# DengZhuangSouthRd/simple_tensorflow

Hardware: AMD Instinct MI355X
Metric: images/sec (higher is better)
Workload: dtype bf16; 1 GPU; model=resnet50_v1, global_batch=256, parallelism=dp1

## Files before the change

simple_tensorflow_amd/csrc/kernels/gpu_conv.cc:

```cpp
#include "kernels/gpu_common.h"

namespace stf {
namespace {

struct GpuConvGeom {
  int64_t N, H, W, C, R, S, K, sh, sw, ph, pw, P, Q;
  int64_t M() const { return N * P * Q; }
  int64_t RSC() const { return R * S * C; }
  int64_t RSCp() const { return (RSC() + 63) & ~int64_t(63); }
  bool is_1x1_s1() const {
    return R == 1 && S == 1 && sh == 1 && sw == 1 && ph == 0 && pw == 0;
  }
  StfConvGeom abi() const {
    return StfConvGeom{(int)N,  (int)H,  (int)W,  (int)C,  (int)R, (int)S,
                       (int)sh, (int)sw, (int)ph, (int)pw, (int)P, (int)Q, K};
  }
};

static Status GetConvGeom(const TensorShape& x, const TensorShape& f,
                          const std::vector<int64_t>& strides,
                          const std::string& padding, GpuConvGeom* g) {
  g->N = x.dim_size(0);
  g->H = x.dim_size(1);
  g->W = x.dim_size(2);
// ... 103 lines not shown
                                        s));
      return;
    }
    if (path == kImplicitNT) {
      OP_HIP_OK(ctx, stf_conv2d_fwd_nt(x.raw_data(), w.raw_data(),
                                       y->raw_data(), ZeroPage(), &sg, rscp,
                                       s));
      return;
    }
    Tensor col = x;
    if (!g.is_1x1_s1()) OP_HIP_OK(ctx, Im2Col(ctx, x, g, rscp, &col, s));
    if (!fits_8ph && (g.K & 7) == 0) {
      OP_HIP_OK(ctx, stf_gemm_bf16(col.raw_data(), w.raw_data(), y->raw_data(),
                                   g.M(), g.K, rscp, rscp, g.K, 0, 1, s));
    } else {
      OP_HIP_OK(ctx, TransposeBf16(ctx, w.raw_data(), rscp, g.K, &wt, s));
      OP_HIP_OK(ctx, stf_gemm_bf16_nt(col.raw_data(), wt.raw_data(),
                                      y->raw_data(), g.M(), g.K, rscp, s));
    }
  }

 private:
  std::vector<int64_t> strides_;
  std::string padding_;
};
REGISTER_KERNEL_BUILDER(Name("Conv2D").Device(DEVICE_GPU).TypeConstraint<bfloat16>("T"), GpuConv2DOp);

class GpuConv2DBackpropInputOp : public OpKernel {
 public:
  explicit GpuConv2DBackpropInputOp(OpKernelConstruction* c, bool side = false)
      : OpKernel(c), side_(side) {
    c->GetAttr("strides", &strides_);
    c->GetAttr("padding", &padding_);
  }
  void Compute(OpKernelContext* ctx) override {
    auto in_sizes = IntVector(ctx->input(0));
    const Tensor& w = ctx->input(1);
    const Tensor& dy = ctx->input(2);
    hipStream_t s = GPU_STREAM(ctx);
    TensorShape x_shape(in_sizes);
    GpuConvGeom g;
    OP_REQUIRES_OK(ctx, GetConvGeom(x_shape, w.shape(), strides_, padding_,
                                    &g));
    Tensor* dx = ctx->allocate_output(0, x_shape);
    const void* side = nullptr;
    if (side_) {
      const Tensor& sd = ctx->input(3);
      OP_REQUIRES(ctx, sd.NumElements() == dx->NumElements(),
                  errors::InvalidArgument(
                      "Conv2DBackpropInputAdd: side shape mismatch"));
      side = sd.raw_data();
    }
    if (g.is_1x1_s1() && side && stf_gemm_bf16_8ph_ok(g.M(), g.RSC(), g.K)) {
      OP_HIP_OK(ctx, stf_gemm_bf16_8ph_side(dy.raw_data(), w.raw_data(),
                                            dx->raw_data(), side, g.M(),
                                            g.RSC(), g.K, g.K, g.K, s));
      return;
    }
    if (g.is_1x1_s1()) {
      OP_HIP_OK(ctx, stf_gemm_bf16_nt(dy.raw_data(), w.raw_data(),
                                      dx->raw_data(), g.M(), g.RSC(), g.K, s));
    } else {
      Tensor dcol = ctx->allocate_temp(DT_BFLOAT16,
                                       TensorShape({g.M(), g.RSC()}));
      OP_HIP_OK(ctx, stf_gemm_bf16_nt(dy.raw_data(), w.raw_data(),
                                      dcol.raw_data(), g.M(), g.RSC(), g.K,
                                      s));
      StfConvGeom sg = g.abi();
      OP_HIP_OK(ctx, stf_col2im_bf16(dcol.raw_data(), dx->raw_data(), &sg, s));
    }
    if (side)
      OP_HIP_OK(ctx, stf_binary(B_ADD, DtypeCode(DT_BFLOAT16), dx->raw_data(),
                                side, dx->raw_data(), dx->NumElements(), s));
  }

 private:
  std::vector<int64_t> strides_;
  std::string padding_;
  bool side_;
};
REGISTER_KERNEL_BUILDER(Name("Conv2DBackpropInput").Device(DEVICE_GPU).TypeConstraint<bfloat16>("T").HostMemory("input_sizes"), GpuConv2DBackpropInputOp);

class GpuConv2DBackpropInputAddOp : public GpuConv2DBackpropInputOp {
 public:
  explicit GpuConv2DBackpropInputAddOp(OpKernelConstruction* c)
      : GpuConv2DBackpropInputOp(c, true) {}
};
REGISTER_KERNEL_BUILDER(Name("Conv2DBackpropInputAdd").Device(DEVICE_GPU).TypeConstraint<bfloat16>("T").HostMemory("input_sizes"), GpuConv2DBackpropInputAddOp);

class GpuConv2DBackpropFilterOp : public OpKernel {
 public:
  explicit GpuConv2DBackpropFilterOp(OpKernelConstruction* c) : OpKernel(c) {
    c->GetAttr("strides", &strides_);
    c->GetAttr("padding", &padding_);
  }
  void Compute(OpKernelContext* ctx) override {
    hipStream_t s = GPU_STREAM(ctx);
    const Tensor& x = ctx->input(0);
    auto f_sizes = IntVector(ctx->input(1));
    const Tensor& dy = ctx->input(2);
    TensorShape f_shape(f_sizes);
    GpuConvGeom g;
    OP_REQUIRES_OK(ctx, GetConvGeom(x.shape(), f_shape, strides_, padding_,
                                    &g));
    Tensor* dw = ctx->allocate_output(0, f_shape);
    int64_t rsc = g.RSC();

    bool pad_c = (g.C % 8) != 0 && x.dtype() == DT_BFLOAT16;
    enum { kImplicit, kKMajorGemm, kTransposeGemm } path =
        ImplicitConvEnabled() && !g.is_1x1_s1() &&
                ((g.C % 8) == 0 || pad_c) && (g.K & 7) == 0 &&
                (g.M() & 63) == 0 && ZeroPage()
// ... 147 lines not shown
```

simple_tensorflow_amd/csrc/kernels/gpu_nn.cc:

```cpp
#include "kernels/gpu_common.h"

namespace stf {
namespace {

class GpuBiasAddOp : public OpKernel {
 public:
  using OpKernel::OpKernel;
  void Compute(OpKernelContext* ctx) override {
    const Tensor& x = ctx->input(0);
    const Tensor& b = ctx->input(1);
    Tensor* y = ctx->allocate_output(0, x.shape());
    OP_HIP_OK(ctx, stf_bias_add(DtypeCode(x.dtype()), x.raw_data(),
                                b.raw_data(), y->raw_data(), x.NumElements(),
                                (int)b.NumElements(), GPU_STREAM(ctx)));
  }
};
REGISTER_KERNEL_BUILDER(Name("BiasAdd").Device(DEVICE_GPU).TypeConstraint<float>("T"), GpuBiasAddOp);
REGISTER_KERNEL_BUILDER(Name("BiasAdd").Device(DEVICE_GPU).TypeConstraint<bfloat16>("T"), GpuBiasAddOp);

class GpuBiasAddGradOp : public OpKernel {
 public:
  using OpKernel::OpKernel;
  void Compute(OpKernelContext* ctx) override {
    const Tensor& dy = ctx->input(0);
// ... 150 lines not shown
                                   offset.raw_data(), y->raw_data(), rows, c,
                                   s));
  }

 private:
  float eps_ = 1e-4f;
};
REGISTER_KERNEL_BUILDER(Name("BatchNormAddReluMi").Device(DEVICE_GPU).TypeConstraint<bfloat16>("T"), GpuBatchNormAddReluMiOp);

class GpuBatchNormMiGradOp : public OpKernel {
 public:
  explicit GpuBatchNormMiGradOp(OpKernelConstruction* c) : OpKernel(c) {
    c->GetAttr("fuse_relu", &fuse_relu_);
  }
  void Compute(OpKernelContext* ctx) override {
    const Tensor& dy = ctx->input(0);
    const Tensor& x = ctx->input(1);
    const Tensor& scale = ctx->input(2);
    const Tensor& mean = ctx->input(3);
    const Tensor& inv_std = ctx->input(4);
    const Tensor& y_relu = ctx->input(5);
    int c = (int)x.dim_size(x.dims() - 1);
    int64_t rows = x.NumElements() / c;
    Tensor* dx = ctx->allocate_output(0, x.shape());
    Tensor* dscale = ctx->allocate_output(1, TensorShape({c}));
    Tensor* doffset = ctx->allocate_output(2, TensorShape({c}));
    hipStream_t s = GPU_STREAM(ctx);
    OP_HIP_OK(ctx, ZeroF32(doffset->raw_data(), c, s));
    OP_HIP_OK(ctx, ZeroF32(dscale->raw_data(), c, s));
    OP_HIP_OK(ctx, stf_bn_bwd(DtypeCode(x.dtype()), dy.raw_data(),
                              x.raw_data(), y_relu.raw_data(),
                              mean.flat<float>(), inv_std.flat<float>(),
                              scale.raw_data(), doffset->flat<float>(),
                              dscale->flat<float>(), dx->raw_data(), rows, c,
                              fuse_relu_ ? 1 : 0, s));
  }

 private:
  bool fuse_relu_ = false;
};
class GpuBatchNormAddReluMiGradOp : public OpKernel {
 public:
  using OpKernel::OpKernel;
  void Compute(OpKernelContext* ctx) override {
    const Tensor& dy = ctx->input(0);
    const Tensor& x = ctx->input(1);
    const Tensor& scale = ctx->input(2);
    const Tensor& mean = ctx->input(3);
    const Tensor& inv_std = ctx->input(4);
    const Tensor& y_relu = ctx->input(5);
    int c = (int)x.dim_size(x.dims() - 1);
    int64_t rows = x.NumElements() / c;
    Tensor* dx = ctx->allocate_output(0, x.shape());
    Tensor* dscale = ctx->allocate_output(1, TensorShape({c}));
    Tensor* doffset = ctx->allocate_output(2, TensorShape({c}));
    Tensor* dside = ctx->allocate_output(3, x.shape());
    hipStream_t s = GPU_STREAM(ctx);
    OP_HIP_OK(ctx, ZeroF32(doffset->raw_data(), c, s));
    OP_HIP_OK(ctx, ZeroF32(dscale->raw_data(), c, s));
    OP_HIP_OK(ctx, stf_bn_bwd(DtypeCode(x.dtype()), dy.raw_data(),
                              x.raw_data(), y_relu.raw_data(),
                              mean.flat<float>(), inv_std.flat<float>(),
                              scale.raw_data(), doffset->flat<float>(),
                              dscale->flat<float>(), dx->raw_data(), rows, c,
                              1, s));
    OP_HIP_OK(ctx, stf_binary(B_RELU_GRAD, DtypeCode(x.dtype()),
                              dy.raw_data(), y_relu.raw_data(),
                              dside->raw_data(), x.NumElements(), s));
  }
};
REGISTER_KERNEL_BUILDER(Name("BatchNormAddReluMiGrad").Device(DEVICE_GPU).TypeConstraint<bfloat16>("T"), GpuBatchNormAddReluMiGradOp);

REGISTER_KERNEL_BUILDER(Name("BatchNormMiGrad").Device(DEVICE_GPU).TypeConstraint<float>("T"), GpuBatchNormMiGradOp);
REGISTER_KERNEL_BUILDER(Name("BatchNormMiGrad").Device(DEVICE_GPU).TypeConstraint<bfloat16>("T"), GpuBatchNormMiGradOp);

struct PoolAttrs {
  std::vector<int64_t> ksize, strides;
  std::string padding;
};
static void GetPool(OpKernelConstruction* c, PoolAttrs* p) {
  c->GetAttr("ksize", &p->ksize);
  c->GetAttr("strides", &p->strides);
  c->GetAttr("padding", &p->padding);
}
static StfPoolGeom PoolGeomFor(const TensorShape& x, const PoolAttrs& p) {
  StfPoolGeom g;
  g.N = (int)x.dim_size(0);
  g.H = (int)x.dim_size(1);
  g.W = (int)x.dim_size(2);
  g.C = (int)x.dim_size(3);
  g.kh = (int)p.ksize[1];
  g.kw = (int)p.ksize[2];
  g.sh = (int)p.strides[1];
  g.sw = (int)p.strides[2];
  if (p.padding == "SAME") {
    g.P = (g.H + g.sh - 1) / g.sh;
    g.Q = (g.W + g.sw - 1) / g.sw;
    g.ph = std::max(0, (g.P - 1) * g.sh + g.kh - g.H) / 2;
    g.pw = std::max(0, (g.Q - 1) * g.sw + g.kw - g.W) / 2;
  } else {
    g.P = (g.H - g.kh) / g.sh + 1;
// ... 185 lines not shown
```

simple_tensorflow_amd/csrc/kernels/hip/bn.hip:

```cpp
#include "hip_common.h"
#include "stf_kernels.h"

namespace {

template <typename T>
__global__ void BnStatsKernel(const T* __restrict__ x, float* __restrict__ acc,
                              int64_t rows, int c) {
  extern __shared__ __attribute__((aligned(16))) char smem[];
  float* s1 = (float*)smem;
  float* s2 = s1 + c;
  for (int i = threadIdx.x; i < c; i += blockDim.x) {
    s1[i] = 0.f;
    s2[i] = 0.f;
  }
  __syncthreads();
  int64_t n = rows * c;
  int64_t gstride = (int64_t)gridDim.x * blockDim.x;
  for (int64_t i = (int64_t)blockIdx.x * blockDim.x + threadIdx.x; i < n;
       i += gstride) {
    float f = (float)x[i];
    int ch = (int)(i % c);
    atomicAdd(&s1[ch], f);
    atomicAdd(&s2[ch], f * f);
  }
// ... 40 lines not shown
                                  const T* __restrict__ x,
                                  const T* __restrict__ yr,
                                  const float* __restrict__ mean,
                                  const float* __restrict__ inv_std,
                                  float* __restrict__ sum_dy,
                                  float* __restrict__ sum_dy_xhat,
                                  int64_t rows, int c) {
  extern __shared__ __attribute__((aligned(16))) char smem[];
  float* s1 = (float*)smem;
  float* s2 = s1 + c;
  for (int i = threadIdx.x; i < c; i += blockDim.x) {
    s1[i] = 0.f;
    s2[i] = 0.f;
  }
  __syncthreads();
  int64_t n = rows * c;
  int64_t gstride = (int64_t)gridDim.x * blockDim.x;
  for (int64_t i = (int64_t)blockIdx.x * blockDim.x + threadIdx.x; i < n;
       i += gstride) {
    int ch = (int)(i % c);
    float gf = (float)dy[i];
    if (RELU && (float)yr[i] <= 0.f) gf = 0.f;
    float xhat = ((float)x[i] - mean[ch]) * inv_std[ch];
    atomicAdd(&s1[ch], gf);
    atomicAdd(&s2[ch], gf * xhat);
  }
  __syncthreads();
  for (int i = threadIdx.x; i < c; i += blockDim.x) {
    atomicAdd(&sum_dy[i], s1[i]);
    atomicAdd(&sum_dy_xhat[i], s2[i]);
  }
}

template <typename T, bool RELU>
__global__ void BnGradKernel(const T* __restrict__ dy, const T* __restrict__ x,
                             const T* __restrict__ yr,
                             const float* __restrict__ mean,
                             const float* __restrict__ inv_std,
                             const float* __restrict__ scale,
                             const float* __restrict__ sum_dy,
                             const float* __restrict__ sum_dy_xhat,
                             T* __restrict__ dx, int64_t n, int64_t rows,
                             int c) {
  int64_t stride = (int64_t)gridDim.x * blockDim.x;
  float inv_rows = 1.f / (float)rows;
  for (int64_t i = blockIdx.x * blockDim.x + threadIdx.x; i < n; i += stride) {
    int ch = (int)(i % c);
    float xhat = ((float)x[i] - mean[ch]) * inv_std[ch];
    float g = (float)dy[i];
    if (RELU && (float)yr[i] <= 0.f) g = 0.f;
    dx[i] = (T)(scale[ch] * inv_std[ch] *
                (g - sum_dy[ch] * inv_rows -
                 xhat * sum_dy_xhat[ch] * inv_rows));
  }
}

struct BnIdx {
  int nw;
  int w;
  int64_t chunk;
  int64_t chunks;
  bool active;
};

__device__ __forceinline__ BnIdx BnThreadIndex(int c, int64_t rows) {
  BnIdx ix;
  ix.nw = c >> 3;
  int64_t tid = (int64_t)blockIdx.x * blockDim.x + threadIdx.x;
  int64_t nthreads = (int64_t)gridDim.x * blockDim.x;
  ix.chunks = nthreads / ix.nw;
  if (ix.chunks > rows) ix.chunks = rows;
  if (ix.chunks < 1) ix.chunks = 1;
  ix.w = (int)(tid % ix.nw);
  ix.chunk = tid / ix.nw;
  ix.active = ix.chunk < ix.chunks;
  return ix;
}

inline int BnGridV9(int c, int64_t rows) {
  int nw = c >> 3;
  int64_t chunks = (131072 + nw - 1) / nw;
  if (chunks > rows) chunks = rows;
  if (chunks < 1) chunks = 1;
  return (int)((nw * chunks + 255) / 256) + 1;
}

// ... 132 lines not shown
    for (int e = 0; e < 8; ++e) {
      mloc[e] = mean[cb + e];
      iloc[e] = inv_std[cb + e];
    }
    int64_t off = (int64_t)cb;
    for (int64_t r = ix.chunk; r < rows; r += ix.chunks) {
      __bf16 g[8], xv[8], yv[8];
      Load8(g, dy + r * c + off);
      Load8(xv, x + r * c + off);
      if (RELU) Load8(yv, yr + r * c + off);
#pragma unroll
      for (int e = 0; e < 8; ++e) {
        float gf = (float)g[e];
        if (RELU && (float)yv[e] <= 0.f) gf = 0.f;
        float xhat = ((float)xv[e] - mloc[e]) * iloc[e];
        p1[e] += gf;
        p2[e] += gf * xhat;
      }
    }
#pragma unroll
    for (int e = 0; e < 8; ++e) {
      atomicAdd(&s1[cb + e], p1[e]);
      atomicAdd(&s2[cb + e], p2[e]);
    }
  }
  __syncthreads();
  for (int i = threadIdx.x; i < c; i += blockDim.x)
    if (s1[i] != 0.f || s2[i] != 0.f) {
      atomicAdd(&sum_dy[i], s1[i]);
      atomicAdd(&sum_dy_xhat[i], s2[i]);
    }
}

template <bool RELU>
__global__ void BnGradKernelV9(const __bf16* __restrict__ dy,
                               const __bf16* __restrict__ x,
                               const __bf16* __restrict__ yr,
                               const float* __restrict__ mean,
                               const float* __restrict__ inv_std,
                               const float* __restrict__ scale,
                               const float* __restrict__ sum_dy,
                               const float* __restrict__ sum_dy_xhat,
                               __bf16* __restrict__ dx, int64_t rows, int c) {
  BnIdx ix = BnThreadIndex(c, rows);
  if (!ix.active) return;
  int cb = ix.w * 8;
  float inv_rows = 1.f / (float)rows;
  float m[8], is[8], k[8], a[8], b[8];
#pragma unroll
  for (int e = 0; e < 8; ++e) {
    m[e] = mean[cb + e];
    is[e] = inv_std[cb + e];
    k[e] = scale[cb + e] * is[e];
    a[e] = sum_dy[cb + e] * inv_rows;
    b[e] = sum_dy_xhat[cb + e] * inv_rows;
  }
  for (int64_t r = ix.chunk; r < rows; r += ix.chunks) {
    __bf16 g8[8], x8[8], y8[8], o[8];
    Load8(g8, dy + r * c + cb);
    Load8(x8, x + r * c + cb);
    if (RELU) Load8(y8, yr + r * c + cb);
#pragma unroll
    for (int e = 0; e < 8; ++e) {
      float xhat = ((float)x8[e] - m[e]) * is[e];
      float g = (float)g8[e];
      if (RELU && (float)y8[e] <= 0.f) g = 0.f;
      o[e] = (__bf16)(k[e] * (g - a[e] - xhat * b[e]));
    }
    Store8(dx + r * c + cb, o);
  }
}

inline bool UseV9(int dtype, int c) { return dtype != 0 && c % 8 == 0; }

inline size_t BnLdsBytes(int c) { return (size_t)c * 2 * sizeof(float); }

void LaunchBnStats(int dtype, const void* x, float* acc, float* mean,
                   float* var, float* inv_std, int64_t rows, int c, float eps,
                   hipStream_t stream) {
  if (UseV9(dtype, c)) {
    hipLaunchKernelGGL(BnStatsKernelV9, dim3(BnGridV9(c, rows)), dim3(256),
                       BnLdsBytes(c), stream, (const __bf16*)x, acc, rows, c);
  } else {
    DispatchDtype(dtype, [&](auto t) {
      using T = typename decltype(t)::type;
      hipLaunchKernelGGL((BnStatsKernel<T>), dim3(512), dim3(256),
                         BnLdsBytes(c), stream, (const T*)x, acc, rows, c);
    });
  }
  hipLaunchKernelGGL(BnFinalizeKernel, dim3((c + 255) / 256), dim3(256), 0,
                     stream, acc, mean, var, inv_std, rows, c, eps);
}

}

extern "C" {

hipError_t stf_bn_stats_only(int dtype, const void* x, float* acc, float* mean,
                             float* var, float* inv_std, int64_t rows, int c,
                             float eps, hipStream_t stream) {
  LaunchBnStats(dtype, x, acc, mean, var, inv_std, rows, c, eps, stream);
  return hipGetLastError();
// ... 11 lines not shown
                         dim3(256), 0, stream, (const __bf16*)x, mean,
                         inv_std, (const float*)scale, (const float*)offset,
                         (__bf16*)y, rows, c);
      return;
    }
    DispatchDtype(dtype, [&](auto t) {
      using T = typename decltype(t)::type;
      int64_t n = rows * c;
      hipLaunchKernelGGL((BnNormKernel<T, RELU>), ElemwiseGrid(n, 256, 4),
                         dim3(256), 0, stream, (const T*)x, mean, inv_std,
                         (const float*)scale, (const float*)offset, (T*)y, n,
                         c);
    });
  });
  return hipGetLastError();
}

hipError_t stf_bn_add_relu(const void* x, const void* side, const float* mean,
                           const float* inv_std, const void* scale,
                           const void* offset, void* y, int64_t rows, int c,
                           hipStream_t stream) {
  if (c % 8 != 0) return hipErrorInvalidValue;
  hipLaunchKernelGGL(BnNormAddReluKernelV9, dim3(BnGridV9(c, rows)),
                     dim3(256), 0, stream, (const __bf16*)x,
                     (const __bf16*)side, mean, inv_std, (const float*)scale,
                     (const float*)offset, (__bf16*)y, rows, c);
  return hipGetLastError();
}

hipError_t stf_bn_bwd(int dtype, const void* dy, const void* x,
                      const void* y_relu, const float* mean,
                      const float* inv_std, const void* scale,
                      float* sum_dy, float* sum_dy_xhat, void* dx,
                      int64_t rows, int c, int fuse_relu,
                      hipStream_t stream) {
  DispatchBool(fuse_relu, [&](auto relu) {
    constexpr bool RELU = decltype(relu)::value;
    if (UseV9(dtype, c)) {
      dim3 g9(BnGridV9(c, rows));
      hipLaunchKernelGGL((BnGradStatsKernelV9<RELU>), g9, dim3(256),
                         BnLdsBytes(c), stream, (const __bf16*)dy,
                         (const __bf16*)x, (const __bf16*)y_relu, mean,
                         inv_std, sum_dy, sum_dy_xhat, rows, c);
      hipLaunchKernelGGL((BnGradKernelV9<RELU>), g9, dim3(256), 0, stream,
                         (const __bf16*)dy, (const __bf16*)x,
                         (const __bf16*)y_relu, mean, inv_std,
                         (const float*)scale, sum_dy, sum_dy_xhat,
                         (__bf16*)dx, rows, c);
      return;
    }
    DispatchDtype(dtype, [&](auto t) {
      using T = typename decltype(t)::type;
      int64_t n = rows * c;
      hipLaunchKernelGGL((BnGradStatsKernel<T, RELU>), dim3(512), dim3(256),
                         BnLdsBytes(c), stream, (const T*)dy, (const T*)x,
                         (const T*)y_relu, mean, inv_std, sum_dy, sum_dy_xhat,
                         rows, c);
      hipLaunchKernelGGL((BnGradKernel<T, RELU>), ElemwiseGrid(n, 256, 4),
                         dim3(256), 0, stream, (const T*)dy, (const T*)x,
                         (const T*)y_relu, mean, inv_std,
                         (const float*)scale, sum_dy, sum_dy_xhat, (T*)dx, n,
                         rows, c);
    });
  });
  return hipGetLastError();
}

}
```

simple_tensorflow_amd/csrc/kernels/hip/conv_im2col.hip:

```cpp
#include "hip_common.h"
#include "stf_kernels.h"

namespace {

struct ConvGeom {
  int N, H, W, C, R, S, K, sh, sw, ph, pw, P, Q;
};

__global__ void Im2ColKernel(const __bf16* __restrict__ x,
                             __bf16* __restrict__ col, ConvGeom g,
                             int64_t total_vec, int vec, int64_t ld) {
  int64_t stride = (int64_t)gridDim.x * blockDim.x;
  int64_t cvec = g.C / vec;
  for (int64_t i = blockIdx.x * blockDim.x + threadIdx.x; i < total_vec;
       i += stride) {
    int64_t rem = i;
    int64_t cv = rem % cvec; rem /= cvec;
    int s = (int)(rem % g.S); rem /= g.S;
    int r = (int)(rem % g.R); rem /= g.R;
    int q = (int)(rem % g.Q); rem /= g.Q;
    int p = (int)(rem % g.P); rem /= g.P;
    int n = (int)rem;
    int ih = p * g.sh - g.ph + r;
    int iw = q * g.sw - g.pw + s;
    int64_t m = ((int64_t)(n * g.P + p) * g.Q + q);
    int64_t rsc = ((int64_t)(r * g.S + s) * g.C + cv * vec);
    __bf16* dst = col + m * ld + rsc;
    if (ih >= 0 && ih < g.H && iw >= 0 && iw < g.W) {
      const __bf16* src =
          x + (((int64_t)(n * g.H + ih) * g.W + iw) * g.C + cv * vec);
      if (vec == 8) {
        *(ulong2*)dst = *(const ulong2*)src;
      } else {
        for (int e = 0; e < vec; ++e) dst[e] = src[e];
      }
    } else {
      if (vec == 8) {
        *(ulong2*)dst = ulong2{0, 0};
      } else {
        for (int e = 0; e < vec; ++e) dst[e] = (__bf16)0.f;
      }
    }
  }
}

__global__ void Col2ImKernel(const __bf16* __restrict__ dcol,
                             __bf16* __restrict__ dx, ConvGeom g,
                             int64_t total) {
  int64_t stride = (int64_t)gridDim.x * blockDim.x;
  int64_t RSC = (int64_t)g.R * g.S * g.C;
  for (int64_t i = blockIdx.x * blockDim.x + threadIdx.x; i < total;
       i += stride) {
    int64_t rem = i;
    int c = (int)(rem % g.C); rem /= g.C;
    int iw = (int)(rem % g.W); rem /= g.W;
    int ih = (int)(rem % g.H); rem /= g.H;
    int n = (int)rem;
    float acc = 0.f;
    for (int r = 0; r < g.R; ++r) {
      int ph = ih + g.ph - r;
      if (ph < 0 || ph % g.sh) continue;
      int p = ph / g.sh;
      if (p >= g.P) continue;
      for (int s = 0; s < g.S; ++s) {
        int pw = iw + g.pw - s;
        if (pw < 0 || pw % g.sw) continue;
        int q = pw / g.sw;
        if (q >= g.Q) continue;
        int64_t m = (int64_t)(n * g.P + p) * g.Q + q;
        acc += (float)dcol[m * RSC + (int64_t)(r * g.S + s) * g.C + c];
      }
    }
    dx[i] = (__bf16)acc;
  }
}

__global__ void Col2ImKernelV8(const __bf16* __restrict__ dcol,
                               __bf16* __restrict__ dx, ConvGeom g,
                               int64_t total8) {
  int64_t stride = (int64_t)gridDim.x * blockDim.x;
  int64_t RSC = (int64_t)g.R * g.S * g.C;
  int cg = g.C / 8;
  for (int64_t i = blockIdx.x * blockDim.x + threadIdx.x; i < total8;
       i += stride) {
    int64_t rem = i;
    int c8 = (int)(rem % cg); rem /= cg;
    int iw = (int)(rem % g.W); rem /= g.W;
    int ih = (int)(rem % g.H); rem /= g.H;
    int n = (int)rem;
    float acc[8] = {0, 0, 0, 0, 0, 0, 0, 0};
    for (int r = 0; r < g.R; ++r) {
      int ph = ih + g.ph - r;
      if (ph < 0 || ph % g.sh) continue;
      int p = ph / g.sh;
      if (p >= g.P) continue;
      for (int s = 0; s < g.S; ++s) {
        int pw = iw + g.pw - s;
        if (pw < 0 || pw % g.sw) continue;
        int q = pw / g.sw;
        if (q >= g.Q) continue;
        int64_t m = (int64_t)(n * g.P + p) * g.Q + q;
        __bf16 v[8];
        *(ulong2*)v = *(const ulong2*)(
            dcol + m * RSC + (int64_t)(r * g.S + s) * g.C + c8 * 8);
#pragma unroll
        for (int e = 0; e < 8; ++e) acc[e] += (float)v[e];
      }
    }
    __bf16 out[8];
#pragma unroll
    for (int e = 0; e < 8; ++e) out[e] = (__bf16)acc[e];
    *(ulong2*)(dx + i * 8) = *(ulong2*)out;
  }
}

}

namespace {
ConvGeom DeviceGeom(const StfConvGeom& g) {
  return ConvGeom{g.n, g.h, g.w, g.c, g.r, g.s, 0, g.sh, g.sw, g.ph, g.pw,
                  g.p, g.q};
}
}

extern "C" hipError_t stf_im2col_bf16(const void* x, void* col,
                                      const StfConvGeom* sg, int64_t ld,
                                      hipStream_t stream) {
  ConvGeom g = DeviceGeom(*sg);
  int vec = (g.C % 8 == 0) ? 8 : 1;
  int64_t total = (int64_t)g.N * g.P * g.Q * g.R * g.S * (g.C / vec);
  hipLaunchKernelGGL(Im2ColKernel, ElemwiseGrid(total, 256, 1), dim3(256), 0,
                     stream, (const __bf16*)x, (__bf16*)col, g, total, vec,
                     ld);
  return hipGetLastError();
}

extern "C" hipError_t stf_col2im_bf16(const void* dcol, void* dx,
                                      const StfConvGeom* sg,
                                      hipStream_t stream) {
  ConvGeom g = DeviceGeom(*sg);
  int64_t total = (int64_t)g.N * g.H * g.W * g.C;
  if (g.C % 8 == 0) {
    int64_t total8 = total / 8;
    hipLaunchKernelGGL(Col2ImKernelV8, ElemwiseGrid(total8, 256, 1),
                       dim3(256), 0, stream, (const __bf16*)dcol,
                       (__bf16*)dx, g, total8);
  } else {
    hipLaunchKernelGGL(Col2ImKernel, ElemwiseGrid(total, 256, 1), dim3(256),
                       0, stream, (const __bf16*)dcol, (__bf16*)dx, g, total);
  }
  return hipGetLastError();
}
```

simple_tensorflow_amd/csrc/kernels/hip/gemm_bf16_8ph.hip:

```cpp
#include "hip_common.h"
#include "stf_kernels.h"

#include <type_traits>

namespace {

__device__ __forceinline__ f32x4 mfma_bf16_8(bf16x8 a, bf16x8 b, f32x4 c) {
  return __builtin_amdgcn_mfma_f32_16x16x32_bf16(a, b, c, 0, 0, 0);
}

__device__ __forceinline__ int Swz8(int r) { return (r ^ (r >> 3)) & 7; }

constexpr int kBM = 256, kBK = 64;
constexpr int kThreads = 512;

template <int ROWS, class AG>
__device__ __forceinline__ void Stage8(const AG& ag, int64_t row0, int64_t k0,
                                       uint16_t* lds_base, int tid) {
#pragma unroll
  for (int p = 0; p < ROWS / 64; ++p) {
    int s = p * kThreads + tid;
    int r = s >> 3;
    int c8 = (s & 7) ^ Swz8(r);
    const uint16_t* g = ag.at(row0 + r, k0 + c8 * 8);
// ... 220 lines not shown
  if (N % 256 == 0) launch(std::integral_constant<int, 4>{});
  else if (N % 128 == 0) launch(std::integral_constant<int, 2>{});
  else launch(std::integral_constant<int, 1>{});
  return hipGetLastError();
}

}

extern "C" {

int stf_gemm_bf16_8ph_ok(int64_t M, int64_t N, int64_t K) {
  return (M % 256 == 0) && (N % 64 == 0) && (K % 64 == 0) && K > 0;
}

hipError_t stf_gemm_bf16_8ph_side(const void* A, const void* B, void* C,
                                  const void* side_bf16, int64_t M, int64_t N,
                                  int64_t K, int64_t lda, int64_t ldb,
                                  hipStream_t stream) {
  if (!stf_gemm_bf16_8ph_ok(M, N, K)) return hipErrorInvalidValue;
  LinearAG ag{(const uint16_t*)A, lda};
  return Launch8Ph(ag, B, C, side_bf16, M, N, K, ldb, stream);
}

hipError_t stf_conv2d_fwd_8ph(const void* x, const void* wt, void* y,
                              const void* zero16, const StfConvGeom* g,
                              int64_t rscp, hipStream_t stream) {
  int64_t M = (int64_t)g->n * g->p * g->q;
  if (!stf_gemm_bf16_8ph_ok(M, g->cout, rscp) || (g->c % 8) != 0)
    return hipErrorInvalidValue;
  return Launch8Ph(MakeConvAG(*g, x, zero16), wt, y, nullptr, M, g->cout,
                   rscp, rscp, stream);
}

}
```

simple_tensorflow_amd/csrc/kernels/hip/hip_common.h:

```cpp
#pragma once

#include <hip/hip_runtime.h>

#include <cstdint>
#include <type_traits>

#include "stf_kernels.h"

#define STF_WAVE 64
#define STF_NUM_XCD 8
#define STF_NUM_CU 256

using f32x4 = __attribute__((ext_vector_type(4))) float;
using f32x16 = __attribute__((ext_vector_type(16))) float;
using bf16x8 = __attribute__((ext_vector_type(8))) __bf16;
using bf16x4 = __attribute__((ext_vector_type(4))) __bf16;
using s16x8 = __attribute__((ext_vector_type(8))) short;

__device__ __forceinline__ float bf16_to_f32(uint16_t v) {
  union { uint32_t u; float f; } c;
  c.u = ((uint32_t)v) << 16;
  return c.f;
}

// ... 90 lines not shown
  __device__ __forceinline__ const uint16_t* at(int64_t row,
                                                int64_t k8) const {
    if (k8 >= rsc) return zero16;
    uint32_t row32 = (uint32_t)row, k32 = (uint32_t)k8;
    uint32_t n = div_pq.div(row32);
    uint32_t pq = div_pq.mod(row32, n);
    uint32_t p = div_q.div(pq);
    uint32_t q = div_q.mod(pq, p);
    uint32_t rs = div_c.div(k32);
    uint32_t c = div_c.mod(k32, rs);
    uint32_t r = div_s.div(rs);
    uint32_t s_ = div_s.mod(rs, r);
    int h = (int)p * sh - ph + (int)r;
    int w = (int)q * sw - pw + (int)s_;
    if (h < 0 || h >= H || w < 0 || w >= W) return zero16;
    return x + ((((int64_t)n * H + h) * W + w) * C + c);
  }
};

inline ConvAG MakeConvAG(const StfConvGeom& g, const void* x,
                         const void* zero16) {
  ConvAG ag;
  ag.x = (const uint16_t*)x;
  ag.zero16 = (const uint16_t*)zero16;
  ag.div_pq.init((uint32_t)(g.p * g.q));
  ag.div_q.init((uint32_t)g.q);
  ag.div_c.init((uint32_t)g.c);
  ag.div_s.init((uint32_t)g.s);
  ag.H = g.h; ag.W = g.w; ag.C = g.c; ag.S = g.s;
  ag.sh = g.sh; ag.sw = g.sw; ag.ph = g.ph; ag.pw = g.pw;
  ag.rsc = (int64_t)g.r * g.s * g.c;
  return ag;
}
```

simple_tensorflow_amd/csrc/kernels/hip/stf_kernels.h:

```cpp
#pragma once

#include <hip/hip_runtime_api.h>

#include <cstdint>

struct StfConvGeom {
  int n, h, w, c;
  int r, s;
  int sh, sw, ph, pw;
  int p, q;
  int64_t cout;
};

struct StfPoolGeom {
  int N, H, W, C, kh, kw, sh, sw, ph, pw, P, Q;
};

constexpr int kStfMaxPermuteRank = 6;

enum StfReduce { STF_REDUCE_SUM = 0, STF_REDUCE_MAX = 1, STF_REDUCE_MIN = 2 };
constexpr float StfReduceIdentity(StfReduce kind) {
  return kind == STF_REDUCE_SUM ? 0.f
         : kind == STF_REDUCE_MAX ? -3.4e38f : 3.4e38f;
}

extern "C" {

hipError_t stf_gemm_bf16(const void* A, const void* B, void* C, int64_t M,
                         int64_t N, int64_t K, int64_t lda, int64_t ldb,
                         int a_km, int b_km, hipStream_t stream);
hipError_t stf_gemm_bf16_nt(const void* A, const void* B, void* C, int64_t M,
                            int64_t N, int64_t K, hipStream_t stream);
hipError_t stf_gemm_bf16_splitk(const void* A, const void* B, void* C_f32,
                                int64_t M, int64_t N, int64_t K, int64_t lda,
                                int64_t ldb, int a_km, int b_km, int splitk,
                                hipStream_t stream);
int stf_gemm_bf16_8ph_ok(int64_t M, int64_t N, int64_t K);
hipError_t stf_gemm_bf16_8ph_side(const void* A, const void* B, void* C,
                                  const void* side_bf16, int64_t M, int64_t N,
                                  int64_t K, int64_t lda, int64_t ldb,
                                  hipStream_t stream);
hipError_t stf_gemm_f32_nt(const void* A, const void* B, void* C, int64_t M,
                           int64_t N, int64_t K, hipStream_t stream);

hipError_t stf_conv2d_fwd_8ph(const void* x, const void* wt, void* y,
                              const void* zero16, const StfConvGeom* g,
                              int64_t rscp, hipStream_t stream);
hipError_t stf_conv2d_fwd_nt(const void* x, const void* w, void* y,
                             const void* zero16, const StfConvGeom* g,
                             int64_t rscp, hipStream_t stream);
hipError_t stf_conv2d_dw_splitk(const void* x, const void* dy, void* dw_f32,
                                const void* zero16, const StfConvGeom* g,
                                int splitk, hipStream_t stream);
hipError_t stf_im2col_bf16(const void* x, void* col, const StfConvGeom* g,
                           int64_t ld, hipStream_t stream);
hipError_t stf_col2im_bf16(const void* dcol, void* dx, const StfConvGeom* g,
                           hipStream_t stream);

hipError_t stf_depthwise_fwd(const void* x, const void* w, void* y,
                             const StfConvGeom* g, int mult,
                             hipStream_t stream);
hipError_t stf_depthwise_bwd_input(const void* dy, const void* w, void* dx,
                                   const StfConvGeom* g, int mult,
                                   hipStream_t stream);
hipError_t stf_depthwise_bwd_filter(const void* x, const void* dy,
                                    float* dw_f32, const StfConvGeom* g,
                                    int mult, hipStream_t stream);

hipError_t stf_unary(int op, int dtype, const void* x, void* y, int64_t n,
                     hipStream_t stream);
hipError_t stf_binary(int op, int dtype, const void* a, const void* b,
                      void* y, int64_t n, hipStream_t stream);
hipError_t stf_binary_scalar(int op, int dtype, const void* a,
                             const void* scalar, void* y, int64_t n,
                             int scalar_left, hipStream_t stream);
hipError_t stf_binary_bcast(int op, int dtype, const void* a, const void* b,
                            void* y, int64_t n, int rank,
                            const int64_t* out_dims, const int64_t* sa,
                            const int64_t* sb, hipStream_t stream);
hipError_t stf_cast(int sdt, int ddt, const void* x, void* y, int64_t n,
                    hipStream_t stream);
hipError_t stf_cast_f32_bf16_zero(void* src_f32, void* dst_bf16, int64_t n,
                                  hipStream_t stream);
hipError_t stf_fill_f32(void* y, float v, int64_t n, int as_bf16,
                        hipStream_t stream);
hipError_t stf_scale(int dtype, const void* x, void* y, int64_t n,
                     float factor, hipStream_t stream);
hipError_t stf_fused_elementwise(int dtype, const void** inputs,
                                 const uint8_t* scalar_flags, int n_in,
                                 const int64_t* prog, int n_prog, void* out,
// ... 1 lines not shown

hipError_t stf_lrn_fwd(const void* x, void* y, int64_t rows, int c,
                       int radius, float bias, float alpha, float beta,
                       hipStream_t stream);

hipError_t stf_bias_add(int dtype, const void* x, const void* bias, void* y,
                        int64_t n, int c, hipStream_t stream);
hipError_t stf_bias_grad(int dtype, const void* dy, void* db_f32,
                         int64_t rows, int c, hipStream_t stream);
hipError_t stf_softmax(int dtype, int log_sm, const void* x, void* y,
                       int64_t rows, int cols, hipStream_t stream);
hipError_t stf_sparse_xent(int dtype, const void* logits, const void* labels,
                           int labels_i32, void* loss_f32, void* backprop,
                           int64_t rows, int cols, hipStream_t stream);
hipError_t stf_xent(int dtype, const void* logits, const void* labels,
                    void* loss_f32, void* backprop, int64_t rows, int cols,
                    hipStream_t stream);

hipError_t stf_bn_fwd(int dtype, const void* x, const void* scale,
                      const void* offset, float* acc, float* mean, float* var,
                      float* inv_std, void* y, int64_t rows, int c, float eps,
                      int fuse_relu, hipStream_t stream);
hipError_t stf_bn_stats_only(int dtype, const void* x, float* acc,
                             float* mean, float* var, float* inv_std,
                             int64_t rows, int c, float eps,
                             hipStream_t stream);
hipError_t stf_bn_add_relu(const void* x, const void* side, const float* mean,
                           const float* inv_std, const void* scale,
                           const void* offset, void* y, int64_t rows, int c,
                           hipStream_t stream);
hipError_t stf_bn_bwd(int dtype, const void* dy, const void* x,
                      const void* y_relu, const float* mean,
                      const float* inv_std, const void* scale, float* sum_dy,
                      float* sum_dy_xhat, void* dx, int64_t rows, int c,
                      int fuse_relu, hipStream_t stream);

hipError_t stf_pool_fwd(int dtype, int is_max, const void* x, void* y,
                        const StfPoolGeom* g, hipStream_t stream);
hipError_t stf_max_pool_bwd(int dtype, const void* x, const void* dy,
                            float* dx_f32, const StfPoolGeom* g,
                            hipStream_t stream);
hipError_t stf_max_pool_bwd_v8(const void* x, const void* dy, void* dx_bf16,
                               const StfPoolGeom* g, hipStream_t stream);
hipError_t stf_avg_pool_bwd(int dtype, const void* dy, void* dx,
                            const StfPoolGeom* g, hipStream_t stream);

hipError_t stf_lstm_gates(int dtype, const void* gates, const void* c_prev,
                          float forget_bias, void* i_out, void* f_out,
                          void* o_out, void* ci_out, void* cs_out,
                          void* co_out, void* h_out, int64_t batch, int H,
                          hipStream_t stream);
hipError_t stf_lstm_gates_grad(int dtype, const void* c_prev, const void* i_,
                               const void* f_, const void* o_,
                               const void* ci_, const void* co_,
                               const void* dh, const void* dcs_next,
                               void* dgates, void* dc_prev, int64_t batch,
                               int H, hipStream_t stream);

hipError_t stf_transpose2d(int elem_size, const void* in, void* out,
                           int64_t rows, int64_t cols, hipStream_t stream);
hipError_t stf_permute(int elem_size, const void* in, void* out, int64_t n,
                       int rank, const int64_t* out_dims,
                       const int64_t* src_strides, hipStream_t stream);
hipError_t stf_block_pad(int dtype, const void* src, void* dst,
                         int64_t nblocks, int64_t in_block, int64_t out_block,
                         hipStream_t stream);
hipError_t stf_strided_copy(int elem_size, int scatter, const void* src,
                            void* dst, int64_t outer, int64_t rows,
// ... 46 lines not shown
```

simple_tensorflow_amd/csrc/runtime/session.cc:

```cpp
#include "runtime/session.h"

#include "gpu/gpu_tracer.h"

#include <algorithm>
#include <atomic>
#include <chrono>
#include <condition_variable>
#include <set>
#include <thread>

#include "graph/graph.h"

namespace stf {

void AddGpuDevices(DeviceMgr* mgr);
void* NewResourceMgr();
void DeleteResourceMgr(void*);

namespace {

std::pair<std::string, int> ParseTensorName(const std::string& s) {
  auto colon = s.rfind(':');
  if (colon != std::string::npos &&
      s.find_first_not_of("0123456789", colon + 1) == std::string::npos &&
      colon + 1 < s.size())
    return {s.substr(0, colon), atoi(s.c_str() + colon + 1)};
  return {s, 0};
}

NodeDef MakeSendRecv(const std::string& op, const std::string& name,
                     DataType dtype, const std::string& tensor_name,
                     const std::string& send_dev, const std::string& recv_dev) {
  NodeDef d;
  d.name = name;
  d.op = op;
  d.attr[op == "_Recv" ? "tensor_type" : "T"] = AttrValue::Type(dtype);
  d.attr["tensor_name"] = AttrValue::S(tensor_name);
  d.attr["send_device"] = AttrValue::S(send_dev);
  d.attr["recv_device"] = AttrValue::S(recv_dev);
  return d;
}

}

DirectSession::DirectSession(bool force_cpu_only, int num_threads) {
  devices_.AddDevice(std::make_unique<ThreadPoolDevice>("/cpu:0"));
  if (!force_cpu_only) AddGpuDevices(&devices_);
  int n = num_threads > 0 ? num_threads
                          : std::max(4u, std::thread::hardware_concurrency());
  pool_ = std::make_unique<ThreadPool>(n);
  resource_mgr_ = NewResourceMgr();
}

DirectSession::~DirectSession() { DeleteResourceMgr(resource_mgr_); }

Status DirectSession::Create(const GraphDef& def) {
  std::lock_guard<std::mutex> l(mu_);
  graph_def_ = def;
  executors_.clear();
  return Status::OK();
}

Status DirectSession::Extend(const GraphDef& def) {
  std::lock_guard<std::mutex> l(mu_);
  for (auto& n : def.node) graph_def_.node.push_back(n);
  executors_.clear();
  return Status::OK();
}

Status DirectSession::GetOrCreateExecutors(
    const std::vector<std::string>& feeds,
    const std::vector<std::string>& fetches,
    const std::vector<std::string>& targets, ExecutorsAndKeys** out) {
  std::string key;
  for (auto& f : feeds) key += f + ",";
  key += "|";
  for (auto& f : fetches) key += f + ",";
  key += "|";
  for (auto& t : targets) key += t + ",";
  {
    std::lock_guard<std::mutex> l(mu_);
    auto it = executors_.find(key);
    if (it != executors_.end()) {
      *out = it->second.get();
      return Status::OK();
    }
  }
// ... 448 lines not shown
    }
    if (val.IsInitialized() && val.mem_space() == MemSpace::DEVICE) {
      Device* dev = devices_.LookUp(it->second);
      Tensor host;
      Status cs = dev->CopyDeviceTensorToHost(val, &host);
      if (!cs.ok()) {
        fetch_status = cs;
        break;
      }
      val = host;
    }
    outputs->push_back(val);
    std::lock_guard<std::mutex> l(prs->mu);
    prs->pending_fetches.erase(fkey);
  }
  bool finished;
  {
    std::lock_guard<std::mutex> l(prs->mu);
    finished = prs->pending_fetches.empty();
  }
  if (!fetch_status.ok() || finished) {
    prs->rendez->StartAbort(errors::Cancelled("partial run finished"));
    {
      std::unique_lock<std::mutex> l(prs->mu);
      prs->cv.wait_for(l, std::chrono::seconds(2),
                       [&]() { return prs->remaining == 0; });
    }
    std::lock_guard<std::mutex> l(mu_);
    partial_runs_.erase(handle);
  }
  return fetch_status;
}

Status DirectSession::Run(
    const std::vector<std::pair<std::string, Tensor>>& feeds,
    const std::vector<std::string>& fetches,
    const std::vector<std::string>& targets, std::vector<Tensor>* outputs,
    StatsCollector* stats, int64_t timeout_ms) {
  std::vector<std::string> feed_names;
  for (auto& f : feeds) feed_names.push_back(f.first);
  ExecutorsAndKeys* ek = nullptr;
  STF_RETURN_IF_ERROR(GetOrCreateExecutors(feed_names, fetches, targets, &ek));

  auto rendez_sp = std::make_shared<Rendezvous>();
  Rendezvous& rendez = *rendez_sp;
  for (auto& f : feeds) {
    auto [name, port] = ParseTensorName(f.first);
    std::string fkey = "feed:" + name + ":" + std::to_string(port);
    auto it = ek->feed_devices.find(fkey);
    if (it == ek->feed_devices.end())
      return errors::Internal("feed not wired: ", f.first);
    STF_RETURN_IF_ERROR(rendez.Send(
        RendezvousKey("client", it->second, fkey, "", 0), f.second, false));
  }

  bool no_io = feeds.empty() && fetches.empty() && stats == nullptr;
  if (no_io && ek->capture_eligible && ek->graph_exec) {
    outputs->clear();
    return ek->capture_device->LaunchCapturedGraph(ek->graph_exec);
  }
  bool do_capture = false;
  Device* capture_dev = nullptr;
  if (no_io && ek->capture_eligible && !ek->capture_broken &&
      ek->graph_exec == nullptr) {
    std::lock_guard<std::mutex> l(mu_);
    if (++ek->plain_runs > 2) {
// ... 203 lines not shown
```

Before: 6174 images/sec.

## Use implicit-GEMM conv backprop-input and fuse side-add and relu-grad into kernels

Stride-1, non-1x1 Conv2DBackpropInput now runs as an implicit GEMM. It builds a flipped, transposed filter and feeds dy through the existing 8-phase conv A-generator, which avoids materialising the im2col dcol buffer and the col2im pass. The col2im fallback now adds the side input inside the kernel instead of calling a separate binary add. BatchNormAddReluMiGrad writes the relu-gradient side output from inside the BN grad kernel instead of a separate elementwise pass. The change also adds a destructor that aborts pending partial runs, which is unrelated to speed.

```diff
diff --git a/simple_tensorflow_amd/csrc/kernels/gpu_conv.cc b/simple_tensorflow_amd/csrc/kernels/gpu_conv.cc
--- a/simple_tensorflow_amd/csrc/kernels/gpu_conv.cc
+++ b/simple_tensorflow_amd/csrc/kernels/gpu_conv.cc
@@ -159,6 +159,7 @@
       : OpKernel(c), side_(side) {
     c->GetAttr("strides", &strides_);
     c->GetAttr("padding", &padding_);
+    implicit_dx_ = getenv("STF_NO_IMPLICIT_DX") == nullptr;
   }
   void Compute(OpKernelContext* ctx) override {
     auto in_sizes = IntVector(ctx->input(0));
@@ -182,6 +183,20 @@
       OP_HIP_OK(ctx, stf_gemm_bf16_8ph_side(dy.raw_data(), w.raw_data(),
                                             dx->raw_data(), side, g.M(),
                                             g.RSC(), g.K, g.K, g.K, s));
+      return;
+    }
+    StfConvGeom sg = g.abi();
+    int64_t nhw = g.N * g.H * g.W;
+    int64_t rskp = (g.R * g.S * g.K + 63) & ~int64_t(63);
+    bool implicit = implicit_dx_ && g.sh == 1 && g.sw == 1 &&
+                    !g.is_1x1_s1() && (g.K % 8) == 0 && ZeroPage();
+    if (implicit && stf_gemm_bf16_8ph_ok(nhw, g.C, rskp)) {
+      Tensor wt = ctx->allocate_temp(DT_BFLOAT16, TensorShape({g.C, rskp}));
+      OP_HIP_OK(ctx, stf_conv_dx_filter(w.raw_data(), wt.raw_data(), (int)g.R,
+                                        (int)g.S, (int)g.C, g.K, rskp, s));
+      OP_HIP_OK(ctx, stf_conv2d_dx_8ph(dy.raw_data(), wt.raw_data(),
+                                       dx->raw_data(), side, ZeroPage(), &sg,
+                                       rskp, s));
       return;
     }
     if (g.is_1x1_s1()) {
@@ -193,8 +208,9 @@
       OP_HIP_OK(ctx, stf_gemm_bf16_nt(dy.raw_data(), w.raw_data(),
                                       dcol.raw_data(), g.M(), g.RSC(), g.K,
                                       s));
-      StfConvGeom sg = g.abi();
-      OP_HIP_OK(ctx, stf_col2im_bf16(dcol.raw_data(), dx->raw_data(), &sg, s));
+      OP_HIP_OK(ctx, stf_col2im_bf16(dcol.raw_data(), side, dx->raw_data(),
+                                     &sg, s));
+      return;
     }
     if (side)
       OP_HIP_OK(ctx, stf_binary(B_ADD, DtypeCode(DT_BFLOAT16), dx->raw_data(),
@@ -205,6 +221,7 @@
   std::vector<int64_t> strides_;
   std::string padding_;
   bool side_;
+  bool implicit_dx_;
 };
 REGISTER_KERNEL_BUILDER(Name("Conv2DBackpropInput").Device(DEVICE_GPU).TypeConstraint<bfloat16>("T").HostMemory("input_sizes"), GpuConv2DBackpropInputOp);
 
diff --git a/simple_tensorflow_amd/csrc/kernels/gpu_nn.cc b/simple_tensorflow_amd/csrc/kernels/gpu_nn.cc
--- a/simple_tensorflow_amd/csrc/kernels/gpu_nn.cc
+++ b/simple_tensorflow_amd/csrc/kernels/gpu_nn.cc
@@ -206,8 +206,8 @@
                               x.raw_data(), y_relu.raw_data(),
                               mean.flat<float>(), inv_std.flat<float>(),
                               scale.raw_data(), doffset->flat<float>(),
-                              dscale->flat<float>(), dx->raw_data(), rows, c,
-                              fuse_relu_ ? 1 : 0, s));
+                              dscale->flat<float>(), dx->raw_data(), nullptr,
+                              rows, c, fuse_relu_ ? 1 : 0, s));
   }
 
  private:
@@ -236,11 +236,8 @@
                               x.raw_data(), y_relu.raw_data(),
                               mean.flat<float>(), inv_std.flat<float>(),
                               scale.raw_data(), doffset->flat<float>(),
-                              dscale->flat<float>(), dx->raw_data(), rows, c,
-                              1, s));
-    OP_HIP_OK(ctx, stf_binary(B_RELU_GRAD, DtypeCode(x.dtype()),
-                              dy.raw_data(), y_relu.raw_data(),
-                              dside->raw_data(), x.NumElements(), s));
+                              dscale->flat<float>(), dx->raw_data(),
+                              dside->raw_data(), rows, c, 1, s));
   }
 };
 REGISTER_KERNEL_BUILDER(Name("BatchNormAddReluMiGrad").Device(DEVICE_GPU).TypeConstraint<bfloat16>("T"), GpuBatchNormAddReluMiGradOp);
diff --git a/simple_tensorflow_amd/csrc/kernels/hip/bn.hip b/simple_tensorflow_amd/csrc/kernels/hip/bn.hip
--- a/simple_tensorflow_amd/csrc/kernels/hip/bn.hip
+++ b/simple_tensorflow_amd/csrc/kernels/hip/bn.hip
@@ -96,7 +96,7 @@
   }
 }
 
-template <typename T, bool RELU>
+template <typename T, bool RELU, bool DSIDE>
 __global__ void BnGradKernel(const T* __restrict__ dy, const T* __restrict__ x,
                              const T* __restrict__ yr,
                              const float* __restrict__ mean,
@@ -104,8 +104,8 @@
                              const float* __restrict__ scale,
                              const float* __restrict__ sum_dy,
                              const float* __restrict__ sum_dy_xhat,
-                             T* __restrict__ dx, int64_t n, int64_t rows,
-                             int c) {
+                             T* __restrict__ dx, T* __restrict__ dside,
+                             int64_t n, int64_t rows, int c) {
   int64_t stride = (int64_t)gridDim.x * blockDim.x;
   float inv_rows = 1.f / (float)rows;
   for (int64_t i = blockIdx.x * blockDim.x + threadIdx.x; i < n; i += stride) {
@@ -116,6 +116,7 @@
     dx[i] = (T)(scale[ch] * inv_std[ch] *
                 (g - sum_dy[ch] * inv_rows -
                  xhat * sum_dy_xhat[ch] * inv_rows));
+    if (DSIDE) dside[i] = (T)((float)yr[i] > 0.f ? (float)dy[i] : 0.f);
   }
 }
 
@@ -314,7 +315,7 @@
     }
 }
 
-template <bool RELU>
+template <bool RELU, bool DSIDE>
 __global__ void BnGradKernelV9(const __bf16* __restrict__ dy,
                                const __bf16* __restrict__ x,
                                const __bf16* __restrict__ yr,
@@ -323,7 +324,9 @@
                                const float* __restrict__ scale,
                                const float* __restrict__ sum_dy,
                                const float* __restrict__ sum_dy_xhat,
-                               __bf16* __restrict__ dx, int64_t rows, int c) {
+                               __bf16* __restrict__ dx,
+                               __bf16* __restrict__ dside, int64_t rows,
+                               int c) {
   BnIdx ix = BnThreadIndex(c, rows);
   if (!ix.active) return;
   int cb = ix.w * 8;
@@ -338,7 +341,7 @@
     b[e] = sum_dy_xhat[cb + e] * inv_rows;
   }
   for (int64_t r = ix.chunk; r < rows; r += ix.chunks) {
-    __bf16 g8[8], x8[8], y8[8], o[8];
+    __bf16 g8[8], x8[8], y8[8], o[8], ds[8];
     Load8(g8, dy + r * c + cb);
     Load8(x8, x + r * c + cb);
     if (RELU) Load8(y8, yr + r * c + cb);
@@ -348,8 +351,10 @@
       float g = (float)g8[e];
       if (RELU && (float)y8[e] <= 0.f) g = 0.f;
       o[e] = (__bf16)(k[e] * (g - a[e] - xhat * b[e]));
+      if (DSIDE) ds[e] = (__bf16)((float)y8[e] > 0.f ? (float)g8[e] : 0.f);
     }
     Store8(dx + r * c + cb, o);
+    if (DSIDE) Store8(dside + r * c + cb, ds);
   }
 }
 
@@ -427,8 +432,9 @@
                       const void* y_relu, const float* mean,
                       const float* inv_std, const void* scale,
                       float* sum_dy, float* sum_dy_xhat, void* dx,
-                      int64_t rows, int c, int fuse_relu,
+                      void* dside, int64_t rows, int c, int fuse_relu,
                       hipStream_t stream) {
+  if (dside && !fuse_relu) return hipErrorInvalidValue;
   DispatchBool(fuse_relu, [&](auto relu) {
     constexpr bool RELU = decltype(relu)::value;
     if (UseV9(dtype, c)) {
@@ -437,11 +443,14 @@
                          BnLdsBytes(c), stream, (const __bf16*)dy,
                          (const __bf16*)x, (const __bf16*)y_relu, mean,
                          inv_std, sum_dy, sum_dy_xhat, rows, c);
-      hipLaunchKernelGGL((BnGradKernelV9<RELU>), g9, dim3(256), 0, stream,
-                         (const __bf16*)dy, (const __bf16*)x,
-                         (const __bf16*)y_relu, mean, inv_std,
-                         (const float*)scale, sum_dy, sum_dy_xhat,
-                         (__bf16*)dx, rows, c);
+      DispatchBool(RELU && dside, [&](auto ds) {
+        constexpr bool DSIDE = RELU && decltype(ds)::value;
+        hipLaunchKernelGGL((BnGradKernelV9<RELU, DSIDE>), g9, dim3(256), 0,
+                           stream, (const __bf16*)dy, (const __bf16*)x,
+                           (const __bf16*)y_relu, mean, inv_std,
+                           (const float*)scale, sum_dy, sum_dy_xhat,
+                           (__bf16*)dx, (__bf16*)dside, rows, c);
+      });
       return;
     }
     DispatchDtype(dtype, [&](auto t) {
@@ -451,11 +460,14 @@
                          BnLdsBytes(c), stream, (const T*)dy, (const T*)x,
                          (const T*)y_relu, mean, inv_std, sum_dy, sum_dy_xhat,
                          rows, c);
-      hipLaunchKernelGGL((BnGradKernel<T, RELU>), ElemwiseGrid(n, 256, 4),
-                         dim3(256), 0, stream, (const T*)dy, (const T*)x,
-                         (const T*)y_relu, mean, inv_std,
-                         (const float*)scale, sum_dy, sum_dy_xhat, (T*)dx, n,
-                         rows, c);
+      DispatchBool(RELU && dside, [&](auto ds) {
+        constexpr bool DSIDE = RELU && decltype(ds)::value;
+        hipLaunchKernelGGL((BnGradKernel<T, RELU, DSIDE>),
+                           ElemwiseGrid(n, 256, 4), dim3(256), 0, stream,
+                           (const T*)dy, (const T*)x, (const T*)y_relu, mean,
+                           inv_std, (const float*)scale, sum_dy, sum_dy_xhat,
+                           (T*)dx, (T*)dside, n, rows, c);
+      });
     });
   });
   return hipGetLastError();
diff --git a/simple_tensorflow_amd/csrc/kernels/hip/conv_im2col.hip b/simple_tensorflow_amd/csrc/kernels/hip/conv_im2col.hip
--- a/simple_tensorflow_amd/csrc/kernels/hip/conv_im2col.hip
+++ b/simple_tensorflow_amd/csrc/kernels/hip/conv_im2col.hip
@@ -45,6 +45,7 @@
 }
 
 __global__ void Col2ImKernel(const __bf16* __restrict__ dcol,
+                             const __bf16* __restrict__ side,
                              __bf16* __restrict__ dx, ConvGeom g,
                              int64_t total) {
   int64_t stride = (int64_t)gridDim.x * blockDim.x;
@@ -71,11 +72,14 @@
         acc += (float)dcol[m * RSC + (int64_t)(r * g.S + s) * g.C + c];
       }
     }
-    dx[i] = (__bf16)acc;
+    __bf16 o = (__bf16)acc;
+    if (side) o = (__bf16)((float)o + (float)side[i]);
+    dx[i] = o;
   }
 }
 
 __global__ void Col2ImKernelV8(const __bf16* __restrict__ dcol,
+                               const __bf16* __restrict__ side,
                                __bf16* __restrict__ dx, ConvGeom g,
                                int64_t total8) {
   int64_t stride = (int64_t)gridDim.x * blockDim.x;
@@ -110,7 +114,36 @@
     __bf16 out[8];
 #pragma unroll
     for (int e = 0; e < 8; ++e) out[e] = (__bf16)acc[e];
+    if (side) {
+      __bf16 sv[8];
+      *(ulong2*)sv = *(const ulong2*)(side + i * 8);
+#pragma unroll
+      for (int e = 0; e < 8; ++e)
+        out[e] = (__bf16)((float)out[e] + (float)sv[e]);
+    }
     *(ulong2*)(dx + i * 8) = *(ulong2*)out;
+  }
+}
+
+__global__ void ConvDxFilterKernel(const __bf16* __restrict__ w,
+                                   __bf16* __restrict__ out, int R, int S,
+                                   int C, int K, int64_t rscp,
+                                   int64_t total8) {
+  int64_t stride = (int64_t)gridDim.x * blockDim.x;
+  int64_t j8n = rscp / 8, rsk = (int64_t)R * S * K;
+  for (int64_t i = blockIdx.x * blockDim.x + threadIdx.x; i < total8;
+       i += stride) {
+    int c = (int)(i / j8n);
+    int64_t j = (i % j8n) * 8;
+    __bf16 v[8];
+    *(ulong2*)v = ulong2{0, 0};
+    if (j < rsk) {
+      int rs = (int)(j / K), k = (int)(j % K);
+      int r = R - 1 - rs / S, s_ = S - 1 - rs % S;
+      *(ulong2*)v =
+          *(const ulong2*)(w + ((int64_t)(r * S + s_) * C + c) * K + k);
+    }
+    *(ulong2*)(out + c * rscp + j) = *(ulong2*)v;
   }
 }
 
@@ -135,8 +168,8 @@
   return hipGetLastError();
 }
 
-extern "C" hipError_t stf_col2im_bf16(const void* dcol, void* dx,
-                                      const StfConvGeom* sg,
+extern "C" hipError_t stf_col2im_bf16(const void* dcol, const void* side,
+                                      void* dx, const StfConvGeom* sg,
                                       hipStream_t stream) {
   ConvGeom g = DeviceGeom(*sg);
   int64_t total = (int64_t)g.N * g.H * g.W * g.C;
@@ -144,10 +177,23 @@
     int64_t total8 = total / 8;
     hipLaunchKernelGGL(Col2ImKernelV8, ElemwiseGrid(total8, 256, 1),
                        dim3(256), 0, stream, (const __bf16*)dcol,
-                       (__bf16*)dx, g, total8);
+                       (const __bf16*)side, (__bf16*)dx, g, total8);
   } else {
     hipLaunchKernelGGL(Col2ImKernel, ElemwiseGrid(total, 256, 1), dim3(256),
-                       0, stream, (const __bf16*)dcol, (__bf16*)dx, g, total);
+                       0, stream, (const __bf16*)dcol, (const __bf16*)side,
+                       (__bf16*)dx, g, total);
   }
   return hipGetLastError();
 }
+
+extern "C" hipError_t stf_conv_dx_filter(const void* w, void* out, int r,
+                                         int s, int c, int64_t k,
+                                         int64_t rscp, hipStream_t stream) {
+  if (k % 8 != 0 || rscp % 8 != 0 || rscp < (int64_t)r * s * k)
+    return hipErrorInvalidValue;
+  int64_t total8 = (int64_t)c * (rscp / 8);
+  hipLaunchKernelGGL(ConvDxFilterKernel, ElemwiseGrid(total8, 256, 1),
+                     dim3(256), 0, stream, (const __bf16*)w, (__bf16*)out, r,
+                     s, c, (int)k, rscp, total8);
+  return hipGetLastError();
+}
diff --git a/simple_tensorflow_amd/csrc/kernels/hip/gemm_bf16_8ph.hip b/simple_tensorflow_amd/csrc/kernels/hip/gemm_bf16_8ph.hip
--- a/simple_tensorflow_amd/csrc/kernels/hip/gemm_bf16_8ph.hip
+++ b/simple_tensorflow_amd/csrc/kernels/hip/gemm_bf16_8ph.hip
@@ -276,4 +276,17 @@
                    rscp, rscp, stream);
 }
 
-}
+hipError_t stf_conv2d_dx_8ph(const void* dy, const void* wt, void* dx,
+                             const void* side, const void* zero16,
+                             const StfConvGeom* g, int64_t rscp,
+                             hipStream_t stream) {
+  int64_t M = (int64_t)g->n * g->h * g->w;
+  if (g->sh != 1 || g->sw != 1 || (g->cout % 8) != 0 ||
+      !stf_gemm_bf16_8ph_ok(M, g->c, rscp) ||
+      rscp < (int64_t)g->r * g->s * g->cout)
+    return hipErrorInvalidValue;
+  return Launch8Ph(MakeConvAG(ConvDxGeom(*g), dy, zero16), wt, dx, side, M,
+                   g->c, rscp, rscp, stream);
+}
+
+}
diff --git a/simple_tensorflow_amd/csrc/kernels/hip/hip_common.h b/simple_tensorflow_amd/csrc/kernels/hip/hip_common.h
--- a/simple_tensorflow_amd/csrc/kernels/hip/hip_common.h
+++ b/simple_tensorflow_amd/csrc/kernels/hip/hip_common.h
@@ -146,3 +146,8 @@
   ag.rsc = (int64_t)g.r * g.s * g.c;
   return ag;
 }
+
+inline StfConvGeom ConvDxGeom(const StfConvGeom& g) {
+  return StfConvGeom{g.n, g.p, g.q, (int)g.cout, g.r, g.s, 1, 1,
+                     g.r - 1 - g.ph, g.s - 1 - g.pw, g.h, g.w, (int64_t)g.c};
+}
diff --git a/simple_tensorflow_amd/csrc/kernels/hip/stf_kernels.h b/simple_tensorflow_amd/csrc/kernels/hip/stf_kernels.h
--- a/simple_tensorflow_amd/csrc/kernels/hip/stf_kernels.h
+++ b/simple_tensorflow_amd/csrc/kernels/hip/stf_kernels.h
@@ -54,8 +54,14 @@
                                 int splitk, hipStream_t stream);
 hipError_t stf_im2col_bf16(const void* x, void* col, const StfConvGeom* g,
                            int64_t ld, hipStream_t stream);
-hipError_t stf_col2im_bf16(const void* dcol, void* dx, const StfConvGeom* g,
-                           hipStream_t stream);
+hipError_t stf_col2im_bf16(const void* dcol, const void* side, void* dx,
+                           const StfConvGeom* g, hipStream_t stream);
+hipError_t stf_conv_dx_filter(const void* w, void* wt, int r, int s, int c,
+                              int64_t k, int64_t rscp, hipStream_t stream);
+hipError_t stf_conv2d_dx_8ph(const void* dy, const void* wt, void* dx,
+                             const void* side, const void* zero16,
+                             const StfConvGeom* g, int64_t rscp,
+                             hipStream_t stream);
 
 hipError_t stf_depthwise_fwd(const void* x, const void* w, void* y,
                              const StfConvGeom* g, int mult,
@@ -123,8 +129,8 @@
 hipError_t stf_bn_bwd(int dtype, const void* dy, const void* x,
                       const void* y_relu, const float* mean,
                       const float* inv_std, const void* scale, float* sum_dy,
-                      float* sum_dy_xhat, void* dx, int64_t rows, int c,
-                      int fuse_relu, hipStream_t stream);
+                      float* sum_dy_xhat, void* dx, void* dside, int64_t rows,
+                      int c, int fuse_relu, hipStream_t stream);
 
 hipError_t stf_pool_fwd(int dtype, int is_max, const void* x, void* y,
                         const StfPoolGeom* g, hipStream_t stream);
diff --git a/simple_tensorflow_amd/csrc/runtime/session.cc b/simple_tensorflow_amd/csrc/runtime/session.cc
--- a/simple_tensorflow_amd/csrc/runtime/session.cc
+++ b/simple_tensorflow_amd/csrc/runtime/session.cc
@@ -51,8 +51,6 @@
   pool_ = std::make_unique<ThreadPool>(n);
   resource_mgr_ = NewResourceMgr();
 }
-
-DirectSession::~DirectSession() { DeleteResourceMgr(resource_mgr_); }
 
 Status DirectSession::Create(const GraphDef& def) {
   std::lock_guard<std::mutex> l(mu_);
@@ -567,6 +565,22 @@
   return fetch_status;
 }
 
+DirectSession::~DirectSession() {
+  std::map<std::string, std::shared_ptr<PartialRunState>> pending;
+  {
+    std::lock_guard<std::mutex> l(mu_);
+    pending.swap(partial_runs_);
+  }
+  for (auto& kv : pending) {
+    PartialRunState& prs = *kv.second;
+    prs.rendez->StartAbort(errors::Cancelled("session closed"));
+    std::unique_lock<std::mutex> l(prs.mu);
+    prs.cv.wait_for(l, std::chrono::seconds(10),
+                    [&]() { return prs.remaining == 0; });
+  }
+  DeleteResourceMgr(resource_mgr_);
+}
+
 Status DirectSession::Run(
     const std::vector<std::pair<std::string, Tensor>>& feeds,
     const std::vector<std::string>& fetches,
```

After: 6697 images/sec, median of 6. 1.08x the previous value.
